# Ladme/groan_rs

Hardware: AMD Instinct MI355X
Metric: frames/sec RMSD-fit, 1e6 atoms triclinic, 1/2/4/8 GPUs; HBM GB/s vs peak (higher is better)
Workload: dtype f32 (fp64 accumulators)

## Files before the change

groan_rs_amd/csrc/gr_api.hip:

```cpp
#include <hip/hip_runtime.h>

#include <cmath>
#include <cstdio>
#include <cstdlib>
#include <cstring>
#include <map>
#include <string>
#include <vector>

#include "../../include/groan_hip.h"
#include "gr_batch.h"
#include "gr_buf.h"
#include "gr_workers.h"
#include "gr_container.h"
#include "gr_kernels.h"
#include "gr_hot.h"
#include "gr_resident.h"
#include "gr_small.h"
#include "gr_xtc.h"
#include "gr_shape.h"
#include "gr_xtc_dev.h"
#include "gr_xtc_enc_dev.h"
#include "gr_trr.h"
#include "gr_cellgrid.h"
// ... 18 lines not shown
    uint32_t *mask_dev = nullptr;
    bool walk_rw = false;
    bool masked = false;
    uint32_t span = 0;
};

}

struct GrWhole;

struct gr_ctx {
    int device = 0;
    hipStream_t stream = nullptr;
    hipStream_t copy_stream = nullptr;
    std::vector<hipEvent_t> ev_ready;
    std::vector<uint8_t> upload_pending;
    hipEvent_t ev_done_ring[64] = {};
    uint64_t done_gen = 0;
    std::vector<uint64_t> slot_gen;
    uint32_t *fuse_cnt = nullptr;
    int fuse = 1;
    uint64_t center_fallbacks = 0;
    uint32_t com_onepass_min = 4096;
    uint64_t n = 0, n_pad = 0;
    uint32_t n_slots = 0;
    size_t frame_stride = 0;
    float *frames = nullptr;
    float *aos_up = nullptr;
    float *aos_dl = nullptr;
    float *masses = nullptr;
    std::vector<float> masses_host;
    GrBox *boxes_dev = nullptr;
    GrBox *boxes_host = nullptr;
    std::vector<int> box_status;
    std::vector<uint8_t> box9_set;
    std::vector<float> box9_host;
    std::map<std::string, Group> groups;
    GrWhole *whole = nullptr;
    GrCenPartial *cen_partials = nullptr;
    GrAccPartial *acc_partials = nullptr;
    grbuf::Dev<double> fit_partials;
    int two_pass = 1;
    int masked_sel = 1;
    int rmsd_fast = 1;
    int rmsd_fast_sigmas = 6;
    uint32_t rmsd_fast_min = 16384;
    uint64_t rmsd_fast_frames = 0, rmsd_exact_redos = 0;
    int resident = 1;
    int pd_sym = 1;
    int res_wg_groups = 0;
    int res_streams = 0;
    int res_fill16 = 1;
    uint32_t res_last_streams = 0;
    int res_metro_ns = 1;
    int stream_wgs_cu = 0;
    int translate_rows = 1;
    int center_resident = 1;
    uint64_t cen_res_launches = 0, cen_res_redone = 0;
    int res_fit_last = 0;
    struct Metro { uint64_t shape = 0; double free_ns = 0, T_ns = 0, best_ns = 0, fail_ns = 0; uint32_t off_for = 0, held = 0; } metro;
    uint64_t res_metro_period_ns = 0, res_last_turn_ns = 0, res_late_permille = 0, res_sclk_mhz = 0;
    int wall_khz = 100000;
    uint32_t res_max_wgs = 0;
    int res_test_no_start = 0;
    uint32_t res_test_abort_at = 0xFFFFFFFFu;
    uint32_t res_skip = 0, res_backoff = 0;
// ... 309 lines not shown
    if (!ingest) return busy_check(c);
    if (c->in_flight && slot < c->in_flight_s0 + c->in_flight_n && c->in_flight_s0 < slot + n)
        return fail(c, GR_E_INVALID_ARG, "upload into a slot of the batch in flight: call gr_rmsd_batch_end first (or use the other half of the double buffer)");
    return GR_OK;
}

struct SlotUse {
    gr_ctx *c; uint32_t first, n;
    bool quiet = false;
    SlotUse(gr_ctx *ctx, uint32_t first_slot, uint32_t count = 1) : c(ctx), first(first_slot), n(count) {
        for (uint32_t s = first; s < first + n && s < c->n_slots; ++s)
            if (c->upload_pending[s]) { (void)hipStreamWaitEvent(c->stream, c->ev_ready[s], 0); c->upload_pending[s] = 0; }
    }
    ~SlotUse() {
        if (quiet) return;
        const uint64_t gen = ++c->done_gen;
        (void)hipEventRecord(c->ev_done_ring[gen % 64], c->stream);
        for (uint32_t s = first; s < first + n && s < c->n_slots; ++s) c->slot_gen[s] = gen;
    }
};

static hipError_t sync_ingest(gr_ctx *c) {
    hipError_t e = hipStreamSynchronize(c->copy_stream);
    if (e == hipSuccess && c->unpack_stream) e = hipStreamSynchronize(c->unpack_stream);
    return e;
}
static int slot_box_wait(gr_ctx *c, uint32_t slot) {
    if (c->ev_ready[slot]) HIPCHK(c, hipEventSynchronize(c->ev_ready[slot]));
    else HIPCHK(c, hipEventCreateWithFlags(&c->ev_ready[slot], hipEventDisableTiming));
    return GR_OK;
}
void box_fill(gr_ctx *c, uint32_t slot, const float *box9) {
    GrBox &b = c->boxes_host[slot];
    if (!box9) {
        gr_box_setup(nullptr, &b);
        c->box_status[slot] = GR_E_NO_BOX; c->box9_set[slot] = 0;
    } else {
        const int ok = gr_box_setup(box9, &b);
        memcpy(&c->box9_host[9 * (size_t)slot], box9, 9 * sizeof(float));
        c->box9_set[slot] = 1;
        if (!ok) c->box_status[slot] = GR_E_ZERO_BOX;
        else if (b.ncand > GR_MAX_CAND) c->box_status[slot] = GR_E_UNSUPPORTED_BOX;
        else c->box_status[slot] = GR_OK;
    }
}
int set_box(gr_ctx *c, uint32_t slot, const float *box9, hipStream_t on = nullptr) {
    box_fill(c, slot, box9);
    HIPCHK(c, hipMemcpyAsync(c->boxes_dev + slot, &c->boxes_host[slot], sizeof(GrBox), hipMemcpyHostToDevice, on ? on : c->stream));
    return GR_OK;
}

int set_boxes_same(gr_ctx *c, uint32_t first_slot, uint32_t n, const float *box9, hipStream_t on = nullptr) {
    if (n == 0) return GR_OK;
    float keep[9];
    if (box9) memcpy(keep, box9, sizeof keep);
    box_fill(c, first_slot, box9 ? keep : nullptr);
    for (uint32_t f = 1; f < n; ++f) {
        const uint32_t s = first_slot + f;
        c->boxes_host[s] = c->boxes_host[first_slot];
        c->box_status[s] = c->box_status[first_slot]; c->box9_set[s] = c->box9_set[first_slot];
        if (box9) memcpy(&c->box9_host[9 * (size_t)s], keep, sizeof keep);
    }
    HIPCHK(c, hipMemcpyAsync(c->boxes_dev + first_slot, c->boxes_host + first_slot, (size_t)n * sizeof(GrBox), hipMemcpyHostToDevice, on ? on : c->stream));
    return GR_OK;
}

int ensure_staging(gr_ctx *c, float **buf) {
    if (*buf) return GR_OK;
    HIPCHK(c, hipMalloc(buf, c->frame_stride * sizeof(float)));
    HIPCHK(c, hipMemsetAsync(*buf, 0, c->frame_stride * sizeof(float), c->stream));
    HIPCHK(c, hipStreamSynchronize(c->stream));
    return GR_OK;
}
int untile_slot(gr_ctx *c, uint32_t slot) {
    int st = ensure_staging(c, &c->aos_dl); if (st) return st;
    const uint32_t ng = (uint32_t)(c->n_pad >> 2);
    k_untile<<<dim3((ng + 255) / 256), dim3(256), 0, c->stream>>>(c->frames + (size_t)slot * c->frame_stride, c->aos_dl, ng);
    HIPCHK(c, hipGetLastError());
    return GR_OK;
}

int ensure_event(gr_ctx *c, hipEvent_t *ev, bool timing) {
    if (*ev) return GR_OK;
    HIPCHK(c, timing ? hipEventCreate(ev) : hipEventCreateWithFlags(ev, hipEventDisableTiming));
    return GR_OK;
}
#define EVREC(ctx, ev, timing, stream) do { int s_ = ensure_event((ctx), &(ev), (timing)); if (s_) return s_; HIPCHK((ctx), hipEventRecord((ev), (stream))); } while (0)

int state_reset(gr_ctx *c, uint32_t n) {
// ... 32 lines not shown
    return GR_OK;
}

static int res_next_epoch(gr_ctx *c, uint32_t *epoch) {
    if (++c->res_epoch == 0u) {
        HIPCHK(c, hipStreamSynchronize(c->stream));
        if (c->res_wgrec.get()) HIPCHK(c, hipMemset(c->res_wgrec.get(), 0, c->res_wgrec.cap() * sizeof(unsigned long long)));
        HIPCHK(c, hipMemset(c->res_rec, 0, (size_t)GR_MAX_BATCH * 16 * sizeof(unsigned long long)));
        HIPCHK(c, hipMemset(c->res_abort + 2, 0, 2 * sizeof(uint32_t)));
        c->res_epoch = 1u;
    }
    *epoch = c->res_epoch;
    return GR_OK;
}
static int res_wgrec_reserve(gr_ctx *c, size_t rec_words, hipStream_t S) {
    bool grew = false;
    HIPCHK(c, c->res_wgrec.reserve(rec_words, grbuf::exact, &grew));
    const hipError_t e = grew ? hipMemsetAsync(c->res_wgrec.get(), 0, rec_words * sizeof(unsigned long long), S) : hipSuccess;
    if (e != hipSuccess) c->res_wgrec.release();
    HIPCHK(c, e);
    return GR_OK;
}
static int res_test_no_start(gr_ctx *c, uint32_t epoch) {
    if (!c->res_test_no_start) return GR_OK;
    const unsigned long long two = 2ull | ((unsigned long long)epoch << 32);
    c->res_test_no_start = 0;
    HIPCHK(c, hipMemcpyAsync(c->res_abort + 2, &two, sizeof two, hipMemcpyHostToDevice, c->stream));
    HIPCHK(c, hipStreamSynchronize(c->stream));
    return GR_OK;
}
template <int MODE>
static int res_close(gr_ctx *c, uint32_t nb, const double *fit_partials, uint32_t nparts, double sum_w, uint32_t epoch, bool fresh, uint32_t *seq) {
    const uint32_t sq = c->res_seq + 1u;
    k_res_close<MODE><<<dim3(nb), dim3(64), 0, c->stream>>>(fit_partials, nparts, sum_w, c->state_dev, c->res_rec, epoch, fresh ? 1u : 0u, c->res_abort, c->res_closed + nb,
                                                        c->res_out_dev->st, c->res_out_dev->words, &c->res_out_dev->seq, sq);
    HIPCHK(c, hipGetLastError());
    c->res_seq = sq; c->res_closed += nb; *seq = sq;
    return GR_OK;
}
static int res_collect(gr_ctx *c, uint32_t seq, uint32_t nb, uint32_t epoch, bool *started) {
    volatile uint32_t *w = &c->res_out->seq;
    const auto t0 = std::chrono::steady_clock::now();
    for (uint32_t spins = 0; *w != seq; ++spins) {
        if ((spins & 1023u) == 1023u && std::chrono::steady_clock::now() - t0 > std::chrono::milliseconds(20)) {
            c->res_sync_fallbacks++;
            HIPCHK(c, hipStreamSynchronize(c->stream));
            if (*w != seq) return fail(c, GR_E_HIP, "the kernel behind the resident pass ended without publishing its results");
            break;
        }
    }
    std::atomic_thread_fence(std::memory_order_acquire);
    memcpy(c->state_host, c->res_out->st, (size_t)nb * sizeof(GrFrameState));
    memcpy(c->res_words_host, c->res_out->words, 12 * sizeof(uint32_t));
    for (int k = 0; k < 2; ++k) { const uint32_t v = c->res_words_host[8 + k]; c->res_words_host[8 + k] = v - c->res_late_seen[k]; c->res_late_seen[k] = v; }
    *started = c->res_words_host[2] == 1u && c->res_words_host[3] == epoch;
    if (!*started || c->res_words_host[0]) HIPCHK(c, hipStreamSynchronize(c->stream));
    return GR_OK;
}

int center_stage(gr_ctx *c, uint32_t first_slot, uint32_t nf, const GrSel &sel, int kind, int weighted,
                 int mass_first, int target, int only_status = 0) {
    if (small_ok(c, sel)) {
        k_center_small_stage<<<dim3(nf), dim3(64), 0, c->stream>>>(c->frames, c->frame_stride, first_slot, c->masses, sel, c->boxes_dev, kind, weighted, mass_first, target, c->state_dev, only_status);
        HIPCHK(c, hipGetLastError());
        return GR_OK;
    }
    uint32_t nch = chunks_for(sel);
    if (nf > 1 && nch >= 8) nch &= ~7u;
// ... 999 lines not shown
    if (!c->center_resident || !csel.contiguous || csel.masked || !all.contiguous || all.start != 0 || all.n != c->n) return GR_OK;
    {
        bool ortho = true;
        for (uint32_t f = 0; f < nb; ++f) if (pre[f] == GR_OK) { ortho = c->boxes_host[s0 + f].ortho != 0; break; }
        if (c->resident == 1 && (uint64_t)csel.n * 100 < c->n * (ortho ? 15u : 3u)) return GR_OK;
    }
    if (small_ok(c, csel)) return GR_OK;
    uint32_t streams = 1, gwg = GR_RES_GROUPS;
    const uint32_t wgs = resident_wgs(c, true, nb, all, &streams, &gwg);
    if (!wgs) return GR_OK;
    if (!resident_acquire(c->device)) return GR_OK;
    struct Release { gr_ctx *c; ~Release() { resident_release(c->device); } } release{ c };
    hipStream_t S = c->stream;
    const uint32_t res_stream = wgs * streams;
    const uint32_t n_fin = std::min<uint32_t>(streams > 8 ? GR_RES_MAX_FIN : 8, c->res_max_wgs - res_stream);
    const size_t rec_words = (size_t)nb * ((wgs + GR_RES_REC_PAD - 1u) & ~(uint32_t)(GR_RES_REC_PAD - 1u)) * GR_RES_REC_WORDS;
    { const int sr = res_wgrec_reserve(c, rec_words, S); if (sr) return sr; }
    GrResCtl ctl;
    memset(&ctl, 0, sizeof ctl);
    { const int se = res_next_epoch(c, &ctl.epoch); if (se) return se; }
    ctl.wgrec = c->res_wgrec.get(); ctl.rec = c->res_rec; ctl.abort = c->res_abort; ctl.progress = c->res_progress; ctl.n_stream = res_stream; ctl.n_fin = n_fin;
    ctl.checkin_target = c->res_checkin + res_stream + n_fin; ctl.fresh_states = fresh_states ? 1u : 0u;
    ctl.wgs_frame = wgs; ctl.streams = streams; ctl.groups_wg = gwg;
    ctl.team_waves = resident_team_waves(wgs, streams);
    ctl.patience_ticks = (unsigned long long)c->wall_khz * 3000ull; ctl.start_ticks = (unsigned long long)c->wall_khz * 200ull;
    ctl.test_abort_frame = c->res_test_abort_at; c->res_test_abort_at = 0xFFFFFFFFu;
    ctl.metro_t16 = c->res_metro_ns >= 100 ? (uint32_t)std::min<uint64_t>(0xFFFFFFFFull, (uint64_t)c->res_metro_ns * (uint64_t)c->wall_khz * 16ull / 1000000ull) : 0u;
    ctl.metro_lead = (uint32_t)((uint64_t)c->wall_khz * 2000ull / 1000000ull);
    ctl.cen_weighted = weighted ? 1u : 0u; ctl.cen_dim_mask = (uint32_t)dim_mask;
    float *frames = c->frames; size_t stride = c->frame_stride; uint32_t slot0 = s0, nfr = nb, natoms = (uint32_t)c->n;
    const float *masses = c->masses; GrSel sel_arg = csel; const GrBox *boxes = c->boxes_dev; GrPlanDev plan; memset(&plan, 0, sizeof plan);
    GrFrameState *states = c->state_dev; double *fparts = nullptr;
    void *args[] = { &frames, &stride, &slot0, &nfr, &natoms, &masses, &sel_arg, &boxes, &plan, &states, &fparts, &ctl };
    bool ubox = true;
    for (uint32_t f = 1; f < nb && ubox; ++f) ubox = memcmp(&c->boxes_host[s0 + f], &c->boxes_host[s0], sizeof(GrBox)) == 0;
    const bool fit_last = c->res_fit_last ? c->res_fit_last == 2 : (uint64_t)res_stream * 10u >= (uint64_t)c->res_max_wgs * 9u;
    { const int sn = res_test_no_start(c, ctl.epoch); if (sn) return sn; }
    if (hipLaunchKernel(resident_center_fn(ubox, fit_last), dim3(res_stream + n_fin), dim3(GrResShape::LANES), args, GrResShape::LDS_BYTES, S) != hipSuccess) {
        (void)hipGetLastError();
        c->res_max_wgs = 0;
        return GR_OK;
    }
    c->res_checkin += res_stream + n_fin;
    uint32_t seq = 0; bool started = false;
    { const int sc = res_close<1>(c, nb, nullptr, 0u, 1.0, ctl.epoch, fresh_states, &seq); if (sc) return sc; }
    { const int sc = res_collect(c, seq, nb, ctl.epoch, &started); if (sc) return sc; }
    c->res_last_streams = streams;
    if (!started) {
        c->res_handshake_misses++;
        c->res_backoff = c->res_backoff ? std::min<uint32_t>(c->res_backoff * 2u, 1024u) : 4u;
        c->res_skip = c->res_backoff;
        return GR_OK;
    }
    c->res_backoff = 0;
    c->cen_res_launches++;
    if (fresh_states) c->res_lean_segments++;
    ran = true;
#ifdef GR_EXP_STEPTIME
    if (getenv("GR_STEPTIME")) {
        unsigned long long st[32];
        if (hipMemcpy(st, c->res_abort + 16, sizeof st, hipMemcpyDeviceToHost) == hipSuccess) {
            const double turns_ = (double)((nb + streams - 1) / streams + GrResShape::K);
            const char *who[4] = { "wg 0 wave 0", "wg 0 wave 5", "wg mid wave 0", "wg mid wave 5" };
            for (int w = 0; w < 4; ++w) {
                fprintf(stderr, "center steptime %-14s ticks/turn:", who[w]);
                double tot = 0; for (int k = 0; k < 7; ++k) tot += (double)st[w * 8 + k];
                const char *nm[7] = { "gate", "request", "rows+sums", "reduce+handover", "record wait", "fit+stores", "park" };
                for (int k = 0; k < 7; ++k) fprintf(stderr, " %s %.0f", nm[k], (double)st[w * 8 + k] / turns_);
// ... 237 lines not shown
    case GR_TUNE_RESIDENT_FIT_LAST: if (value < 0 || value > 2) break; c->res_fit_last = (int)value; return GR_OK;
    case GR_TUNE_STREAM_WGS_PER_CU: if (value < 0 || value > 8) break; c->stream_wgs_cu = (int)value; return GR_OK;
    case GR_TUNE_CENTER_RESIDENT: if (value < 0 || value > 1) break; c->center_resident = (int)value; return GR_OK;
    case GR_TUNE_TRANSLATE_ROWS: if (value < 0 || value > 1) break; c->translate_rows = (int)value; return GR_OK;
    case GR_TUNE_RESIDENT_FILL: if (value < 1 || value > 16) break; c->res_fill16 = (int)value; return GR_OK;
    case GR_TUNE_RESIDENT_GROUPS: if (value != 2) break; return GR_OK;
    case GR_TUNE_TEST_RESIDENT_NO_START: c->res_test_no_start = value ? 1 : 0; return GR_OK;
    case GR_TUNE_TEST_RESIDENT_ABORT_AT: c->res_test_abort_at = value < 0 ? 0xFFFFFFFFu : (uint32_t)value; return GR_OK;
    default: break;
    }
    return fail(c, GR_E_INVALID_ARG, "unknown tuning key or value out of range");
} catch (...) { return gr_abi_guard(); }

static int rmsd_exact(gr_rmsd_plan *p, gr_ctx *c, const GrSel &sel, uint32_t first_slot, uint32_t nf, int fit) {
    int st = pbc_center_stages(c, first_slot, nf, sel, 1); if (st) return st;
    if (small_ok(c, sel)) {
        k_rmsd_small<1><<<dim3(nf), dim3(64), 0, c->stream>>>(c->frames, c->frame_stride, first_slot, c->masses, sel, c->boxes_dev, p->dev, c->state_dev, 1, nullptr, nullptr, 0u);
    } else {
        const uint32_t nch = chunks_for(sel);
        k_rmsd_accum<1><<<dim3(nch, nf), dim3(GR_WG), 0, c->stream>>>(c->frames, c->frame_stride, first_slot, c->masses, sel, c->boxes_dev, p->dev, c->state_dev, c->acc_partials);
        k_rmsd_finalize<1><<<dim3(nf), dim3(GR_WG), 0, c->stream>>>(c->acc_partials, nch, c->frames, c->frame_stride, first_slot, sel, c->boxes_dev, p->dev, c->state_dev);
    }
    if (fit) {
        const uint32_t gx = (uint32_t)std::min<uint64_t>(((c->n >> 2) + GR_WG * 4 - 1) / (GR_WG * 4) + 1, 1024);
        k_fit_pk<false><<<dim3(gx, nf), dim3(GR_WG), 0, c->stream>>>(c->frames, c->frame_stride, first_slot, (uint32_t)c->n, c->boxes_dev, p->dev, c->state_dev, c->masses, sel, nullptr);
    }
    HIPCHK(c, hipGetLastError());
    return GR_OK;
}

static int segment_begin(gr_rmsd_plan *p, uint32_t s0, uint32_t nb, int fit) {
    gr_ctx *c = p->target;
    Pending &q = p->pend;
    q = Pending();
    q.s0 = s0; q.nb = nb; q.fit = fit; q.active = true;
    SlotUse use(c, s0, nb);
    const Group *g = find_group(c, p->group.c_str());
    q.pre.assign(nb, GR_OK); q.pre_idx.assign(nb, 0); q.pre_msg.assign(nb, std::string());
    for (uint32_t f = 0; f < nb; ++f) {
        int s = box_check(c, s0 + f);
        if (s == GR_OK && !g) s = fail(c, GR_E_GROUP_NOT_FOUND, p->group);
        if (s == GR_OK && g->n == 0) s = fail(c, GR_E_EMPTY_GROUP, p->group);
        q.pre[f] = s;
        if (s != GR_OK) { q.pre_msg[f] = c->err; q.pre_idx[f] = c->err_index; }
        q.any_ok = q.any_ok || s == GR_OK;
    }
    if (!q.any_ok) return GR_OK;
    const GrSel sel = make_sel(*g);
    q.sel = sel; q.group_n = g->n; q.has_group = true;
    if (!p->resolved || p->resolved_epoch != c->epoch) {
        p->resolved_epoch = c->epoch;
        bool same = (g->n == p->n_ref);
        if (same) { size_t k = 0; for (uint64_t i : grc::expand(g->blocks)) { const float a = c->masses_host[i], b = p->w_host[k++]; if (!(a == b)) { same = false; break; } } }
        p->dev.w_is_mass = same ? 1u : 0u; p->resolved = true;
        p->span_ok = p->p_span_dev != nullptr && g->masked && g->mask_dev != nullptr && g->blocks == p->ref_blocks;
    }
    q.consistent = (g->n == p->n_ref);
    const bool fast_asked = c->two_pass && c->rmsd_fast && p->dev.w_is_mass != 0 && g->n >= c->rmsd_fast_min && ((!fit && sel.contiguous) || (sel.masked && p->span_ok));
    const bool small = q.consistent && !p->exact && small_ok(c, sel) && !fast_asked;
    if (small && nb == 1) {
        q.small = true; q.small_seq = ++c->small_seq;
        k_rmsd_small<0><<<dim3(1), dim3(64), 0, c->stream>>>(c->frames, c->frame_stride, s0, c->masses, sel, c->boxes_dev, p->dev,
                                                         c->state_dev, 0, c->small_state_dev, c->small_flag_dev, q.small_seq);
        if (fit) k_fit_pk<false><<<dim3(fit_grid(c, 1), 1), dim3(GR_WG), 0, c->stream>>>(c->frames, c->frame_stride, s0, (uint32_t)c->n, c->boxes_dev, p->dev, c->state_dev, c->masses, sel, nullptr);
        p->fit_behind_small = fit != 0;
        HIPCHK(c, hipGetLastError());
        return GR_OK;
    }
    bool states_unset = false;
    {
        bool all_ok = true;
        for (uint32_t f = 0; f < nb; ++f) all_ok = all_ok && q.pre[f] == GR_OK;
        states_unset = all_ok;
        if (!all_ok) {
            for (uint32_t f = 0; f < nb; ++f) { GrFrameState z = {}; z.err_index = GR_NOIDX; z.status = q.pre[f]; c->state_host[f] = z; }
            HIPCHK(c, hipMemcpyAsync(c->state_dev, c->state_host, nb * sizeof(GrFrameState), hipMemcpyHostToDevice, c->stream));
        }
    }
    auto zero_states = [&]() -> int { if (!states_unset) return GR_OK; states_unset = false; return state_reset(c, nb); };
    int st;
    if (!(q.consistent && !p->exact && !small)) { st = zero_states(); if (st) return st; }
    if (small) {
        k_rmsd_small<0><<<dim3(nb), dim3(64), 0, c->stream>>>(c->frames, c->frame_stride, s0, c->masses, sel, c->boxes_dev, p->dev, c->state_dev, 1, nullptr, nullptr, 0u);
        if (fit) k_fit_pk<false><<<dim3(fit_grid(c, nb), nb), dim3(GR_WG), 0, c->stream>>>(c->frames, c->frame_stride, s0, (uint32_t)c->n, c->boxes_dev, p->dev, c->state_dev, c->masses, sel, nullptr);
        HIPCHK(c, hipGetLastError());
    } else if (!q.consistent) {
        st = pbc_center_stages(c, s0, nb, sel, 1); if (st) return st;
    } else if (p->exact) {
        st = rmsd_exact(p, c, sel, s0, nb, fit); if (st) return st;
    } else {
        const uint32_t sb = c->sub_batch;
        const bool lite = fit && sel.contiguous && c->two_pass;
        const bool msk = sel.masked && p->span_ok;
        const bool fast = c->two_pass && c->rmsd_fast && p->dev.w_is_mass != 0 && g->n >= c->rmsd_fast_min && ((!fit && sel.contiguous) || msk);
        q.rmsd_fast = fast;
        p->dev.fast_sigmas = (float)c->rmsd_fast_sigmas;
        GrPlanDev plan_span = p->dev; plan_span.p = p->p_span_dev;
        const uint32_t n_groups = (nb + sb - 1) / sb;
        if (lite) {
            size_t need = 0;
            for (uint32_t f0 = 0; f0 < nb; f0 += sb) need = std::max(need, (size_t)nb * fit_grid(c, std::min<uint32_t>(sb, nb - f0)) * (GR_WG / 64));
            HIPCHK(c, c->fit_partials.reserve(need, grbuf::exact));
        }
        const bool fused = (lite || fast) && c->fuse;
        q.fused = fused;
// ... 24 lines not shown
                if (c->res_metro_ns >= 100) period_ns = (uint32_t)c->res_metro_ns;
                else if (c->res_metro_ns == 0) {
                    gr_ctx::Metro &m = c->metro;
                    if (m.shape != shape) { m = gr_ctx::Metro(); m.shape = shape; }
                    if (m.off_for) m.off_for--;
                    else if (m.free_ns > 0) period_ns = (uint32_t)(m.T_ns + 0.5);
                    q.res_metro_auto = true;
                }
                q.res_metro_ns = period_ns;
                ctl.metro_t16 = (uint32_t)std::min<uint64_t>(0xFFFFFFFFull, (uint64_t)period_ns * (uint64_t)c->wall_khz * 16ull / 1000000ull);
                ctl.metro_lead = (uint32_t)((uint64_t)c->wall_khz * 2000ull / 1000000ull);
            }
#ifdef GR_EXP_STEPTIME
            {
                static unsigned long long *dbg_dev = nullptr;
                if (!dbg_dev) (void)hipMalloc(&dbg_dev, (size_t)GR_MAX_CHUNKS * 8 * 4 * sizeof(unsigned long long));
                ctl.dbg = getenv("GR_STEPTIME") ? dbg_dev : nullptr;
                g_steptime_dbg = ctl.dbg;
            }
#endif
#ifdef GR_EXP_TIMELINE
            {
                static unsigned long long *tl_dev = nullptr; static size_t tl_cap = 0;
                if (nb > tl_cap) { if (tl_dev) (void)hipFree(tl_dev); tl_dev = nullptr; tl_cap = 0; if (hipMalloc(&tl_dev, (size_t)nb * 8 * sizeof(unsigned long long)) == hipSuccess) tl_cap = nb; }
                ctl.tl = getenv("GR_TIMELINE") ? tl_dev : nullptr;
                if (ctl.tl) HIPCHK(c, hipMemsetAsync(ctl.tl, 0, (size_t)nb * 8 * sizeof(unsigned long long), S));
                q.tl_dev = ctl.tl;
            }
#endif
            float *frames = c->frames; size_t stride = c->frame_stride; uint32_t slot0 = s0, nfr = nb, natoms = (uint32_t)c->n;
            const float *masses = c->masses; GrSel sel_arg = sel; const GrBox *boxes = c->boxes_dev; GrPlanDev plan = res_msk ? plan_span : p->dev;
            GrFrameState *states = c->state_dev; double *fparts = c->fit_partials.get();
            void *args[] = { &frames, &stride, &slot0, &nfr, &natoms, &masses, &sel_arg, &boxes, &plan, &states, &fparts, &ctl };
            bool ubox = true;
            for (uint32_t f = 1; f < nb && ubox; ++f) ubox = memcmp(&c->boxes_host[s0 + f], &c->boxes_host[s0], sizeof(GrBox)) == 0;
#ifdef GR_EXP_NO_UBOX
            ubox = false;
#endif
            const bool whole = sel.start == 0 && sel.n == c->n;
            const bool fit_last = c->res_fit_last ? c->res_fit_last == 2 : (uint64_t)res_stream * 10u >= (uint64_t)c->res_max_wgs * 9u;
            const void *fn = resident_fn(p->dev.w_is_mass != 0, ubox, whole, fit_last);
            const uint32_t lanes = GrResShape::LANES, lds = GrResShape::LDS_BYTES;
            st = res_test_no_start(c, ctl.epoch); if (st) return st;
            if (c->profile) EVREC(c, c->pev[0], true, S);
            const hipError_t le = hipLaunchKernel(fn, dim3(res_stream + n_fin), dim3(lanes), args, lds, S);
            if (le == hipSuccess) {
                if (c->profile) EVREC(c, c->pev[1], true, S);
                c->res_checkin += res_stream + n_fin;
                q.res_fresh = states_unset; q.res_epoch = ctl.epoch;
                states_unset = false;
                st = res_close<0>(c, nb, c->fit_partials.get(), res_wgs * GrResShape::WAVES, p->dev.sw, ctl.epoch, q.res_fresh, &q.res_seq); if (st) return st;
                q.resident = true; q.res_stream = res_stream; q.res_streams = res_streams;
                q.rmsd_fast = false;
                c->res_last_streams = res_streams;
            } else {
                (void)hipGetLastError();
                c->res_max_wgs = 0;
                resident_done(c);
            }
        }
        if (!q.resident) { st = zero_states(); if (st) return st; }
        for (uint32_t g = 0; g < n_groups && !q.resident; ++g) {
            const uint32_t f0 = g * sb, nf = std::min<uint32_t>(sb, nb - f0), nch = batch_chunks(c, sel, nf), gx = fit_grid(c, nf);
            GrAccPartial *parts = c->acc_partials + (size_t)f0 * GR_MAX_CHUNKS;
            if (c->profile) EVREC(c, c->pev[6 * g], true, S);
            if (lite) k_sums_pk<false><<<dim3(nch, nf), dim3(GR_WG), 0, S>>>(c->frames, c->frame_stride, s0 + f0, c->masses, sel, c->boxes_dev, p->dev, parts,
                                                                             fused ? c->fuse_cnt + f0 : nullptr, c->state_dev + f0);
            else if (fast && msk) k_sums_pk<false, true, true><<<dim3(nch, nf), dim3(GR_WG), 0, S>>>(c->frames, c->frame_stride, s0 + f0, c->masses, sel, c->boxes_dev, plan_span, parts,
// ... 180 lines not shown
                        const double next = T * 0.985;
                        if (m.fail_ns == 0 || next > m.fail_ns * 1.004) m.T_ns = next;
                        else if (m.best_ns > m.free_ns * 0.98) {
                            m.off_for = 512; m.free_ns = 0; m.T_ns = 0; m.best_ns = 0; m.fail_ns = 0;
                        }
                        else if (++m.held >= 64) { m.held = 0; m.fail_ns *= 0.995; }
                    } else {
                        m.fail_ns = std::max(m.fail_ns, T);
                        m.T_ns = m.best_ns > T ? m.best_ns : T * 1.02;
                        if (m.best_ns > 0 && m.best_ns <= T) m.best_ns = 0;
                        if (m.T_ns >= m.free_ns * 0.995) {
                            m.off_for = 512; m.free_ns = 0; m.T_ns = 0; m.best_ns = 0; m.fail_ns = 0;
                        }
                    }
                }
            }
            if (c->profile) {
                float ms = 0.f;
                hipError_t ee = hipEventElapsedTime(&ms, c->pev[0], c->pev[1]);
                if (ee == hipErrorNotReady) { (void)hipGetLastError(); HIPCHK(c, hipEventSynchronize(c->pev[1])); ee = hipEventElapsedTime(&ms, c->pev[0], c->pev[1]); }
                HIPCHK(c, ee);
                c->prof_ms[3] += ms; c->prof_launches[3] += 1; c->prof_frames[3] += nb;
            }
        }
        for (uint32_t gi = 0; gi < q.n_prof_groups; ++gi) {
            const uint32_t nf = std::min<uint32_t>(c->sub_batch, nb - gi * c->sub_batch);
            for (int k = 0; k < 3; ++k) {
                if ((k == 1 && q.fused) || (k == 2 && !fit)) continue;
                float ms = 0.f;
                HIPCHK(c, hipEventElapsedTime(&ms, c->pev[6 * gi + 2 * k], c->pev[6 * gi + 2 * k + 1]));
                c->prof_ms[k] += ms; c->prof_launches[k] += 1; c->prof_frames[k] += nf;
            }
        }
        std::vector<GrFrameState> res(c->state_host, c->state_host + nb);
        if (!redo.empty()) {
            const int keep = c->resident;
            c->resident = 0;
            int st_redo = GR_OK;
            for (uint32_t f0 = 0; f0 < nb && st_redo == GR_OK; ) {
                if (!redo[f0]) { ++f0; continue; }
                uint32_t f1 = f0;
                while (f1 < nb && redo[f1]) ++f1;
                std::vector<GrFrameState> fs2;
                Pending sub;
                std::swap(sub, p->pend);
                st_redo = segment_begin(p, s0 + f0, f1 - f0, fit);
                if (st_redo == GR_OK) {
                    const int st_nested = segment_end(p, nullptr, nullptr, nullptr, &fs2);
                    if (fs2.size() != (size_t)(f1 - f0)) st_redo = st_nested != GR_OK ? st_nested : GR_E_HIP;
                    else for (uint32_t f = f0; f < f1; ++f) res[f] = fs2[f - f0];
                } else { p->pend.active = false; resident_done(c); }
                std::swap(sub, p->pend);
                c->res_redone_frames += f1 - f0;
                f0 = f1;
            }
            c->resident = keep;
            if (st_redo != GR_OK) return st_redo;
        }
        if (q.rmsd_fast) {
            for (uint32_t f0 = 0; f0 < nb; ) {
                if (res[f0].status != GR_ST_REDO_EXACT) { if (q.pre[f0] == GR_OK) c->rmsd_fast_frames++; ++f0; continue; }
                uint32_t f1 = f0;
                while (f1 < nb && res[f1].status == GR_ST_REDO_EXACT) ++f1;
                const uint32_t nf = f1 - f0, nch = batch_chunks(c, sel, nf);
                SlotUse use(c, s0 + f0, nf);
                int st = state_reset(c, nf); if (st) return st;
                GrAccPartial *parts = c->acc_partials;
// ... 8 lines not shown
                for (uint32_t f = f0; f < f1; ++f) res[f] = c->state_host[f - f0];
                c->rmsd_exact_redos += nf;
                f0 = f1;
            }
        }
        for (uint32_t f0 = 0; f0 < nb; ) {
            if (res[f0].status != GR_ST_FALLBACK || (!redo.empty() && redo[f0])) { ++f0; continue; }
            uint32_t f1 = f0;
            while (f1 < nb && res[f1].status == GR_ST_FALLBACK && (redo.empty() || !redo[f1])) ++f1;
            const uint32_t nf = f1 - f0;
            p->last_fallbacks += nf;
            SlotUse use(c, s0 + f0, nf);
            int st = state_reset(c, nf); if (st) return st;
            st = rmsd_exact(p, c, sel, s0 + f0, nf, fit); if (st) return st;
            st = fetch_states(c, nf); if (st) return st;
            for (uint32_t f = f0; f < f1; ++f) res[f] = c->state_host[f - f0];
            f0 = f1;
        }
        for (uint32_t f = 0; f < nb; ++f) {
            int s = res[f].status;
            if (q.pre[f] != GR_OK) { s = q.pre[f]; c->err = q.pre_msg[f]; c->err_index = q.pre_idx[f]; }
            else if (!torn.empty() && torn[f]) s = fail(c, GR_E_HIP, "the resident RMSD-fit pass stalled while this frame was being fitted: some of its atoms carry the fitted coordinates, others the original ones (frame index in gr_last_error_index)", f);
            else if (s == GR_OK && !q.consistent) {
                c->counts[0] = p->n_ref; c->counts[1] = q.group_n;
                s = fail(c, GR_E_INCONSISTENT_GROUP, p->group);
            } else if (s != GR_OK) {
                s = frame_status(c, res[f]);
            }
            fe.note(c, s);
            if (status_out) status_out[f] = s;
            if (rmsd_out) rmsd_out[f] = (s == GR_OK) ? res[f].rmsd : NAN;
            if (R_out) for (int k = 0; k < 9; ++k) R_out[9 * (size_t)f + k] = (s == GR_OK) ? res[f].R[k] : NAN;
        }
        if (final_states) *final_states = res;
    }
    return fe.finish(c);
}

static int rmsd_batch_impl(gr_rmsd_plan *p, uint32_t first_slot, uint32_t n_frames, float *rmsd_out, int *status_out, float *R_out, int fit) {
    if (!p || !p->target) return GR_E_INVALID_ARG;
    gr_ctx *c = p->target;
    int st = slot_check(c, first_slot, n_frames); if (st) return st;
    (void)hipSetDevice(c->device);
    if (p->pend.active) return fail(c, GR_E_INVALID_ARG, "a batch begun with gr_rmsd_batch_begin is still in flight");
    p->last_fallbacks = 0;
    grb::FirstError<gr_ctx> fe;
    for (const auto [b0, nb, s0] : grb::Segments{ first_slot, n_frames }) {
        st = segment_begin(p, s0, nb, fit);
        if (st) { p->pend.active = false; resident_done(c); return st; }
        st = segment_end(p, rmsd_out ? rmsd_out + b0 : nullptr, status_out ? status_out + b0 : nullptr, R_out ? R_out + 9 * (size_t)b0 : nullptr);
        if (st == GR_E_HIP) return st;
        fe.note(c, st);
    }
    return fe.finish(c);
}

int gr_rmsd_batch_begin(gr_rmsd_plan *p, uint32_t first_slot, uint32_t n, int fit) try {
    if (!p || !p->target) return GR_E_INVALID_ARG;
    gr_ctx *c = p->target;
    int st = slot_check(c, first_slot, n); if (st) return st;
    if (n > GR_MAX_BATCH) return fail(c, GR_E_INVALID_ARG, "at most 1024 frames per asynchronous batch");
    if (p->pend.active) return fail(c, GR_E_INVALID_ARG, "a batch is already in flight on this plan");
    (void)hipSetDevice(c->device);
    p->last_fallbacks = 0;
    st = segment_begin(p, first_slot, n, fit ? 1 : 0);
    if (st) { p->pend.active = false; resident_done(c); } else { c->in_flight = p; c->in_flight_s0 = first_slot; c->in_flight_n = n; }
    return st;
// ... 923 lines not shown
```

groan_rs_amd/csrc/gr_resident.h:

```cpp
#pragma once
#include <type_traits>
#include "gr_hot.h"

struct GrResShape {
    static constexpr int LANES = 512, WAVES = LANES / 64;
#ifndef GR_RES_K
#define GR_RES_K 6
#endif
    static constexpr int K = GR_RES_K;
    static constexpr int R = 8;
    static constexpr int PARK_F4 = K * 3 * LANES;
    static constexpr int WSUM_F = R * WAVES * 32;
#ifdef GR_EXP_TIMELINE
    static constexpr int TL_BYTES = 128 * 4 * 8;
#else
    static constexpr int TL_BYTES = 0;
#endif
    static constexpr int LDS_BYTES = PARK_F4 * 16 + WSUM_F * 4 + R * WAVES * 8 + 3 * R * 4 + 2 * WAVES * 4 + TL_BYTES;
    static constexpr int REC_PER_WAVE = 256 / WAVES, LANES_PER_REC = 64 / REC_PER_WAVE, WORDS_PER_LANE = 32 / LANES_PER_REC;
};
#ifndef GR_RES_SLEEP
#define GR_RES_SLEEP 2
#endif
#ifndef GR_RES_BAL
// ... 912 lines not shown
        ctl.progress[wg_all * WAVES + wave] = n_fitted;
        (void)__hip_atomic_fetch_max(reinterpret_cast<unsigned long long *>(ctl.abort + 6), (unsigned long long)wall_clock64(), __ATOMIC_RELAXED, __HIP_MEMORY_SCOPE_AGENT);
        if (n_late) (void)__hip_atomic_fetch_add(ctl.abort + 8, n_late, __ATOMIC_RELAXED, __HIP_MEMORY_SCOPE_AGENT);
        if (n_waited) (void)__hip_atomic_fetch_add(ctl.abort + 9, n_waited, __ATOMIC_RELAXED, __HIP_MEMORY_SCOPE_AGENT);
#ifdef GR_EXP_STEPTIME
        if (ctl.dbg) {
            unsigned long long *o = ctl.dbg + (size_t)(wg_all * WAVES + wave) * 4u;
            unsigned long long tot = 0; for (int k = 0; k < 7; ++k) tot += st_acc[k];
            o[0] = st_acc[4]; o[1] = st_acc[7] | (st_combines << 32);
            o[2] = (__builtin_amdgcn_s_getreg((20 << 0) | (0 << 6) | (3 << 11)) & 7u) | (simd_of[wave] << 8);
            o[3] = tot;
        }
        if ((wg_all == 0u || wg_all == ctl.n_stream / 2u) && (wave == 0u || wave == 5u)) {
            unsigned long long *o = reinterpret_cast<unsigned long long *>(ctl.abort + 16) + ((wg_all ? 2u : 0u) + (wave ? 1u : 0u)) * 8u;
            for (int k = 0; k < 8; ++k) o[k] = st_acc[k];
        }
#endif
        if (clk_wave) {
            const unsigned long long dc = (unsigned long long)clock64() - clk_c0, dw = (unsigned long long)wall_clock64() - clk_w0;
            gr_st_agent(ctl.abort + 10, (uint32_t)(dc >> 8)); gr_st_agent(ctl.abort + 11, (uint32_t)(dw >> 8));
        }
    }
#ifdef GR_EXP_TIMELINE
    if (tl_wg && wave == 0 && !bail) {
        for (uint32_t t = (n_turns > 128u ? n_turns - 128u : 0u) + lane; t < n_turns; t += 64u) {
            const size_t f = kf(t);
            ctl.tl[f * 8 + 0] = tls[(t & 127u) * 4u + 0u];
            ctl.tl[f * 8 + 6] = tls[(t & 127u) * 4u + 1u] | (tls[(t & 127u) * 4u + 2u] << 48);
        }
    }
#endif
}

template <int MODE>
__global__ __launch_bounds__(64) void k_res_close(const double *__restrict__ fit_partials, uint32_t nparts, double sum_w, GrFrameState *state,
                                                  const unsigned long long *__restrict__ rec, uint32_t epoch, uint32_t fresh_states, uint32_t *ctl_words,
                                                  uint32_t done_target, GrFrameState *out_states, uint32_t *out_words, uint32_t *out_seq, uint32_t seq) {
    constexpr uint32_t NW = sizeof(GrFrameState) / 4u, W_RMSD = offsetof(GrFrameState, rmsd) / 4u, W_STATUS = offsetof(GrFrameState, status) / 4u;
    static_assert(sizeof(GrFrameState) % 4u == 0 && NW <= 64u, "a frame state is exported by one wave, a word per lane");
    const uint32_t frame = blockIdx.x, lane = threadIdx.x;
    uint32_t *sw = reinterpret_cast<uint32_t *>(state + frame);
    uint32_t w = 0u;
    if (fresh_states && (uint32_t)(gr_ld_agent(rec + (size_t)frame * 16u) >> 32) != epoch) {
        GrFrameState z = {};
        z.err_index = GR_NOIDX; z.status = GR_ST_ABORTED;
        if (lane < NW) { w = reinterpret_cast<const uint32_t *>(&z)[lane]; sw[lane] = w; }
    } else if (lane < NW) w = sw[lane];
    const int status = __shfl((int)w, (int)W_STATUS, 64);
    if (MODE == 0 && status == 0) {
        double s0 = 0.0, s1 = 0.0, s2 = 0.0, s3 = 0.0;
        const double *p = fit_partials + (size_t)frame * nparts;
        uint32_t k = lane;
        for (; k + 192 < nparts; k += 256) { s0 += p[k]; s1 += p[k + 64]; s2 += p[k + 128]; s3 += p[k + 192]; }
        for (; k < nparts; k += 64) s0 += p[k];
        const double s = gr_wave_sum((s0 + s1) + (s2 + s3));
        float r = 0.0f;
        if (lane == 0) { r = (float)sqrt(fmax(s, 0.0) / sum_w); state[frame].rmsd = r; }
        r = __shfl(r, 0, 64);
        if (lane == W_RMSD) w = __float_as_uint(r);
    }
    if (lane < NW) reinterpret_cast<uint32_t *>(out_states + frame)[lane] = w;
    __threadfence_system();
    uint32_t n = 0u;
    if (lane == 0) n = __hip_atomic_fetch_add(ctl_words + 12, 1u, __ATOMIC_ACQ_REL, __HIP_MEMORY_SCOPE_AGENT) + 1u;
    n = (uint32_t)__builtin_amdgcn_readfirstlane((int)n);
    if (n != done_target) return;
    if (lane < 12u) out_words[lane] = gr_ld_agent(ctl_words + lane);
    __threadfence_system();
    if (lane == 0) __hip_atomic_store(out_seq, seq, __ATOMIC_RELEASE, __HIP_MEMORY_SCOPE_SYSTEM);
}
```

Measured before the change: 139,500.

## Batch resident close kernel over frames and trim host-side per-segment bookkeeping

The close kernel now packs several frames per block, one wave per frame. It preloads the fit partials in unrolled rounds and does a single atomic per block. The last block copies all frame states to the host-visible buffer in one wide pass instead of each wave writing its own state. On the host, the uniform-box check is cached by a box generation counter, per-frame error vectors are allocated only when an error occurs, and the state vector is copied only when a redo or fallback needs it. These cut launch and host work per batch, at the cost of a serial copy tail in one wave and more complex synchronisation.

```diff
diff --git a/groan_rs_amd/csrc/gr_api.hip b/groan_rs_amd/csrc/gr_api.hip
--- a/groan_rs_amd/csrc/gr_api.hip
+++ b/groan_rs_amd/csrc/gr_api.hip
@@ -74,6 +74,8 @@
     std::vector<float> masses_host;
     GrBox *boxes_dev = nullptr;
     GrBox *boxes_host = nullptr;
+    uint64_t box_gen = 1;
+    struct { uint64_t gen = 0; uint32_t s0 = 0, n = 0; bool same = false; } box_run;
     std::vector<int> box_status;
     std::vector<uint8_t> box9_set;
     std::vector<float> box9_host;
@@ -449,6 +451,7 @@
 }
 void box_fill(gr_ctx *c, uint32_t slot, const float *box9) {
     GrBox &b = c->boxes_host[slot];
+    c->box_gen++;
     if (!box9) {
         gr_box_setup(nullptr, &b);
         c->box_status[slot] = GR_E_NO_BOX; c->box9_set[slot] = 0;
@@ -461,6 +464,14 @@
         else c->box_status[slot] = GR_OK;
     }
 }
+static bool uniform_boxes(gr_ctx *c, uint32_t s0, uint32_t n) {
+    auto &r = c->box_run;
+    if (r.gen == c->box_gen && r.s0 == s0 && r.n == n) return r.same;
+    bool same = true;
+    for (uint32_t f = 1; f < n && same; ++f) same = memcmp(&c->boxes_host[s0 + f], &c->boxes_host[s0], sizeof(GrBox)) == 0;
+    r.gen = c->box_gen; r.s0 = s0; r.n = n; r.same = same;
+    return same;
+}
 int set_box(gr_ctx *c, uint32_t slot, const float *box9, hipStream_t on = nullptr) {
     box_fill(c, slot, box9);
     HIPCHK(c, hipMemcpyAsync(c->boxes_dev + slot, &c->boxes_host[slot], sizeof(GrBox), hipMemcpyHostToDevice, on ? on : c->stream));
@@ -472,6 +483,7 @@
     float keep[9];
     if (box9) memcpy(keep, box9, sizeof keep);
     box_fill(c, first_slot, box9 ? keep : nullptr);
+    c->box_gen++;
     for (uint32_t f = 1; f < n; ++f) {
         const uint32_t s = first_slot + f;
         c->boxes_host[s] = c->boxes_host[first_slot];
@@ -570,8 +582,9 @@
 template <int MODE>
 static int res_close(gr_ctx *c, uint32_t nb, const double *fit_partials, uint32_t nparts, double sum_w, uint32_t epoch, bool fresh, uint32_t *seq) {
     const uint32_t sq = c->res_seq + 1u;
-    k_res_close<MODE><<<dim3(nb), dim3(64), 0, c->stream>>>(fit_partials, nparts, sum_w, c->state_dev, c->res_rec, epoch, fresh ? 1u : 0u, c->res_abort, c->res_closed + nb,
-                                                        c->res_out_dev->st, c->res_out_dev->words, &c->res_out_dev->seq, sq);
+    k_res_close<MODE><<<dim3((nb + GR_RES_CLOSE_WAVES - 1u) / GR_RES_CLOSE_WAVES), dim3(64 * GR_RES_CLOSE_WAVES), 0, c->stream>>>(
+        fit_partials, nparts, sum_w, c->state_dev, c->res_rec, epoch, fresh ? 1u : 0u, c->res_abort, c->res_closed + nb, nb,
+        c->res_out_dev->st, c->res_out_dev->words, &c->res_out_dev->seq, sq);
     HIPCHK(c, hipGetLastError());
     c->res_seq = sq; c->res_closed += nb; *seq = sq;
     return GR_OK;
@@ -1637,8 +1650,7 @@
     const float *masses = c->masses; GrSel sel_arg = csel; const GrBox *boxes = c->boxes_dev; GrPlanDev plan; memset(&plan, 0, sizeof plan);
     GrFrameState *states = c->state_dev; double *fparts = nullptr;
     void *args[] = { &frames, &stride, &slot0, &nfr, &natoms, &masses, &sel_arg, &boxes, &plan, &states, &fparts, &ctl };
-    bool ubox = true;
-    for (uint32_t f = 1; f < nb && ubox; ++f) ubox = memcmp(&c->boxes_host[s0 + f], &c->boxes_host[s0], sizeof(GrBox)) == 0;
+    const bool ubox = uniform_boxes(c, s0, nb);
     const bool fit_last = c->res_fit_last ? c->res_fit_last == 2 : (uint64_t)res_stream * 10u >= (uint64_t)c->res_max_wgs * 9u;
     { const int sn = res_test_no_start(c, ctl.epoch); if (sn) return sn; }
     if (hipLaunchKernel(resident_center_fn(ubox, fit_last), dim3(res_stream + n_fin), dim3(GrResShape::LANES), args, GrResShape::LDS_BYTES, S) != hipSuccess) {
@@ -1942,18 +1954,24 @@
 static int segment_begin(gr_rmsd_plan *p, uint32_t s0, uint32_t nb, int fit) {
     gr_ctx *c = p->target;
     Pending &q = p->pend;
-    q = Pending();
+    {
+        std::vector<int> pre = std::move(q.pre); std::vector<uint64_t> pre_idx = std::move(q.pre_idx); std::vector<std::string> pre_msg = std::move(q.pre_msg);
+        q = Pending();
+        q.pre = std::move(pre); q.pre_idx = std::move(pre_idx); q.pre_msg = std::move(pre_msg);
+    }
     q.s0 = s0; q.nb = nb; q.fit = fit; q.active = true;
     SlotUse use(c, s0, nb);
     const Group *g = find_group(c, p->group.c_str());
-    q.pre.assign(nb, GR_OK); q.pre_idx.assign(nb, 0); q.pre_msg.assign(nb, std::string());
+    q.pre.assign(nb, GR_OK); q.pre_idx.clear(); q.pre_msg.clear();
+    bool all_ok = true;
     for (uint32_t f = 0; f < nb; ++f) {
         int s = box_check(c, s0 + f);
         if (s == GR_OK && !g) s = fail(c, GR_E_GROUP_NOT_FOUND, p->group);
         if (s == GR_OK && g->n == 0) s = fail(c, GR_E_EMPTY_GROUP, p->group);
-        q.pre[f] = s;
-        if (s != GR_OK) { q.pre_msg[f] = c->err; q.pre_idx[f] = c->err_index; }
-        q.any_ok = q.any_ok || s == GR_OK;
+        if (s != GR_OK) {
+            if (all_ok) { q.pre_idx.assign(nb, 0); q.pre_msg.resize(nb); all_ok = false; }
+            q.pre[f] = s; q.pre_msg[f] = c->err; q.pre_idx[f] = c->err_index;
+        } else q.any_ok = true;
     }
     if (!q.any_ok) return GR_OK;
     const GrSel sel = make_sel(*g);
@@ -1979,8 +1997,6 @@
     }
     bool states_unset = false;
     {
-        bool all_ok = true;
-        for (uint32_t f = 0; f < nb; ++f) all_ok = all_ok && q.pre[f] == GR_OK;
         states_unset = all_ok;
         if (!all_ok) {
             for (uint32_t f = 0; f < nb; ++f) { GrFrameState z = {}; z.err_index = GR_NOIDX; z.status = q.pre[f]; c->state_host[f] = z; }
@@ -2071,8 +2087,7 @@
             const float *masses = c->masses; GrSel sel_arg = sel; const GrBox *boxes = c->boxes_dev; GrPlanDev plan = res_msk ? plan_span : p->dev;
             GrFrameState *states = c->state_dev; double *fparts = c->fit_partials.get();
             void *args[] = { &frames, &stride, &slot0, &nfr, &natoms, &masses, &sel_arg, &boxes, &plan, &states, &fparts, &ctl };
-            bool ubox = true;
-            for (uint32_t f = 1; f < nb && ubox; ++f) ubox = memcmp(&c->boxes_host[s0 + f], &c->boxes_host[s0], sizeof(GrBox)) == 0;
+            bool ubox = uniform_boxes(c, s0, nb);
 #ifdef GR_EXP_NO_UBOX
             ubox = false;
 #endif
@@ -2319,7 +2334,11 @@
                 c->prof_ms[k] += ms; c->prof_launches[k] += 1; c->prof_frames[k] += nf;
             }
         }
-        std::vector<GrFrameState> res(c->state_host, c->state_host + nb);
+        bool redo_due = !redo.empty() || q.rmsd_fast || final_states != nullptr;
+        for (uint32_t f = 0; f < nb && !redo_due; ++f) redo_due = c->state_host[f].status == GR_ST_FALLBACK;
+        std::vector<GrFrameState> res_copy;
+        if (redo_due) res_copy.assign(c->state_host, c->state_host + nb);
+        GrFrameState *const res = redo_due ? res_copy.data() : c->state_host;
         if (!redo.empty()) {
             const int keep = c->resident;
             c->resident = 0;
@@ -2394,7 +2413,7 @@
             if (rmsd_out) rmsd_out[f] = (s == GR_OK) ? res[f].rmsd : NAN;
             if (R_out) for (int k = 0; k < 9; ++k) R_out[9 * (size_t)f + k] = (s == GR_OK) ? res[f].R[k] : NAN;
         }
-        if (final_states) *final_states = res;
+        if (final_states) *final_states = std::move(res_copy);
     }
     return fe.finish(c);
 }
diff --git a/groan_rs_amd/csrc/gr_resident.h b/groan_rs_amd/csrc/gr_resident.h
--- a/groan_rs_amd/csrc/gr_resident.h
+++ b/groan_rs_amd/csrc/gr_resident.h
@@ -968,39 +968,82 @@
 #endif
 }
 
+#ifndef GR_RES_CLOSE_WAVES
+#define GR_RES_CLOSE_WAVES 8
+#endif
+#define GR_RES_CLOSE_UNROLL 16
+#define GR_RES_CLOSE_ROUND 32u
 template <int MODE>
-__global__ __launch_bounds__(64) void k_res_close(const double *__restrict__ fit_partials, uint32_t nparts, double sum_w, GrFrameState *state,
+__global__ __launch_bounds__(64 * GR_RES_CLOSE_WAVES) void k_res_close(const double *__restrict__ fit_partials, uint32_t nparts, double sum_w, GrFrameState *state,
                                                   const unsigned long long *__restrict__ rec, uint32_t epoch, uint32_t fresh_states, uint32_t *ctl_words,
-                                                  uint32_t done_target, GrFrameState *out_states, uint32_t *out_words, uint32_t *out_seq, uint32_t seq) {
-    constexpr uint32_t NW = sizeof(GrFrameState) / 4u, W_RMSD = offsetof(GrFrameState, rmsd) / 4u, W_STATUS = offsetof(GrFrameState, status) / 4u;
-    static_assert(sizeof(GrFrameState) % 4u == 0 && NW <= 64u, "a frame state is exported by one wave, a word per lane");
-    const uint32_t frame = blockIdx.x, lane = threadIdx.x;
-    uint32_t *sw = reinterpret_cast<uint32_t *>(state + frame);
-    uint32_t w = 0u;
-    if (fresh_states && (uint32_t)(gr_ld_agent(rec + (size_t)frame * 16u) >> 32) != epoch) {
-        GrFrameState z = {};
-        z.err_index = GR_NOIDX; z.status = GR_ST_ABORTED;
-        if (lane < NW) { w = reinterpret_cast<const uint32_t *>(&z)[lane]; sw[lane] = w; }
-    } else if (lane < NW) w = sw[lane];
-    const int status = __shfl((int)w, (int)W_STATUS, 64);
-    if (MODE == 0 && status == 0) {
-        double s0 = 0.0, s1 = 0.0, s2 = 0.0, s3 = 0.0;
+                                                  uint32_t done_target, uint32_t nb, GrFrameState *__restrict__ out_states, uint32_t *__restrict__ out_words,
+                                                  uint32_t *out_seq, uint32_t seq) {
+    constexpr uint32_t NW = sizeof(GrFrameState) / 4u, W_STATUS = offsetof(GrFrameState, status) / 4u,
+                       W_ERR = offsetof(GrFrameState, err_index) / 4u, WPG = GR_RES_CLOSE_WAVES;
+    static_assert(sizeof(GrFrameState) % 8u == 0 && alignof(GrFrameState) <= 8u && NW <= 64u, "a wave holds a frame state a word per lane; the states are copied in 8-byte words");
+    const uint32_t wave = threadIdx.x >> 6, lane = threadIdx.x & 63u, frame = blockIdx.x * WPG + wave;
+    if (frame < nb) {
+        constexpr uint32_t RW = GR_RES_CLOSE_ROUND;
+        uint32_t *sw = reinterpret_cast<uint32_t *>(state + frame);
         const double *p = fit_partials + (size_t)frame * nparts;
-        uint32_t k = lane;
-        for (; k + 192 < nparts; k += 256) { s0 += p[k]; s1 += p[k + 64]; s2 += p[k + 128]; s3 += p[k + 192]; }
-        for (; k < nparts; k += 64) s0 += p[k];
-        const double s = gr_wave_sum((s0 + s1) + (s2 + s3));
-        float r = 0.0f;
-        if (lane == 0) { r = (float)sqrt(fmax(s, 0.0) / sum_w); state[frame].rmsd = r; }
-        r = __shfl(r, 0, 64);
-        if (lane == W_RMSD) w = __float_as_uint(r);
-    }
-    if (lane < NW) reinterpret_cast<uint32_t *>(out_states + frame)[lane] = w;
-    __threadfence_system();
+        double v[RW];
+        const unsigned long long tag = fresh_states ? gr_ld_agent(rec + (size_t)frame * 16u) : 0ull;
+        uint32_t w = lane < NW ? sw[lane] : 0u;
+        if (MODE == 0) {
+#pragma unroll
+            for (uint32_t j = 0; j < RW; ++j) v[j] = nparts ? p[min(lane + 64u * j, nparts - 1u)] : 0.0;
+        }
+        if (fresh_states && (uint32_t)(tag >> 32) != epoch) {
+            w = lane == W_STATUS ? (uint32_t)GR_ST_ABORTED : lane == W_ERR ? GR_NOIDX : 0u;
+            if (lane < NW) sw[lane] = w;
+        }
+        const int status = __shfl((int)w, (int)W_STATUS, 64);
+        if (MODE == 0 && status == 0) {
+            double s0 = 0.0, s1 = 0.0, s2 = 0.0, s3 = 0.0;
+            for (uint32_t k = lane;;) {
+                const uint32_t r = k < nparts ? min(RW, (nparts - k + 63u) >> 6) : 0u, r4 = r & ~3u;
+#pragma unroll
+                for (uint32_t j = 0; j < RW; j += 4u) {
+                    if (j < r4) { s0 += v[j]; s1 += v[j + 1u]; s2 += v[j + 2u]; s3 += v[j + 3u]; }
+                    else { if (j < r) s0 += v[j]; if (j + 1u < r) s0 += v[j + 1u]; if (j + 2u < r) s0 += v[j + 2u]; }
+                }
+                k += 64u * RW;
+                if (k >= nparts) break;
+#pragma unroll
+                for (uint32_t j = 0; j < RW; ++j) v[j] = p[min(k + 64u * j, nparts - 1u)];
+            }
+            const double s = gr_wave_sum((s0 + s1) + (s2 + s3));
+            if (lane == 0) state[frame].rmsd = (float)sqrt(fmax(s, 0.0) / sum_w);
+        }
+    }
+    uint32_t add = 1u;
+    if (WPG > 1u) {
+        asm volatile("s_waitcnt vmcnt(0)" ::: "memory");
+        __syncthreads();
+        if (wave != 0u) return;
+        add = min(WPG, nb - blockIdx.x * WPG);
+    }
     uint32_t n = 0u;
-    if (lane == 0) n = __hip_atomic_fetch_add(ctl_words + 12, 1u, __ATOMIC_ACQ_REL, __HIP_MEMORY_SCOPE_AGENT) + 1u;
+    if (lane == 0) n = __hip_atomic_fetch_add(ctl_words + 12, add, __ATOMIC_ACQ_REL, __HIP_MEMORY_SCOPE_AGENT) + add;
     n = (uint32_t)__builtin_amdgcn_readfirstlane((int)n);
     if (n != done_target) return;
+    const unsigned long long *src = reinterpret_cast<const unsigned long long *>(state);
+    const uint32_t n8 = nb * (uint32_t)(sizeof(GrFrameState) / 8u), n16 = n8 >> 1;
+    uint4 *dst = reinterpret_cast<uint4 *>(out_states);
+    for (uint32_t base = 0; base < n16; base += 64u * GR_RES_CLOSE_UNROLL) {
+        unsigned long long a[GR_RES_CLOSE_UNROLL], b[GR_RES_CLOSE_UNROLL];
+#pragma unroll
+        for (uint32_t u = 0; u < GR_RES_CLOSE_UNROLL; ++u) {
+            const uint32_t i = min(base + u * 64u + lane, n16 - 1u);
+            a[u] = gr_ld_agent(src + 2u * (size_t)i); b[u] = gr_ld_agent(src + 2u * (size_t)i + 1u);
+        }
+#pragma unroll
+        for (uint32_t u = 0; u < GR_RES_CLOSE_UNROLL; ++u) {
+            const uint32_t i = base + u * 64u + lane;
+            if (i < n16) dst[i] = make_uint4((uint32_t)a[u], (uint32_t)(a[u] >> 32), (uint32_t)b[u], (uint32_t)(b[u] >> 32));
+        }
+    }
+    if ((n8 & 1u) && lane == 0) reinterpret_cast<unsigned long long *>(out_states)[n8 - 1u] = gr_ld_agent(src + n8 - 1u);
     if (lane < 12u) out_words[lane] = gr_ld_agent(ctl_words + lane);
     __threadfence_system();
     if (lane == 0) __hip_atomic_store(out_seq, seq, __ATOMIC_RELEASE, __HIP_MEMORY_SCOPE_SYSTEM);
```

After: 142,400, median of 6. About the same (+2.1%).
